# skipperro/selkies-gstreamer

Hardware: AMD Instinct MI355X
Metric: encoded fps + glass-to-glass p50 ms at 1920x1080; concurrent 60fps sessions/node (higher is better)
Workload: dtype uint8 pixels / int32 integer transforms (bit-exact vs CPU reference); 1 GPU; model=H.264 Constrained Baseline CAVLC, striped stripes 64px, CRF 25, global_batch=8, seq_len=1, parallelism=session-parallel dp1 x 8 sessions/GPU, resolution=1920x1080, backend=hip, deblock=auto, me_full=True, upload_overlap=False, frames_in_flight=1, num_refs=1, numa_node_rank0=0

## Files before the change

csrc/kernels/h264_kernels.hip:

```cpp
#include "h264_gpu.h"
#include "../codec/color.h"
#include "../codec/h264_mb.h"
#include "../codec/h264_ep.h"

namespace sk {
namespace h264 {
namespace gpu {

__device__ __forceinline__ int lane_id() { return threadIdx.x & 63; }

__device__ __forceinline__ void wave_sync() {
    __builtin_amdgcn_fence(__ATOMIC_RELEASE, "wavefront");
    __builtin_amdgcn_wave_barrier();
    __builtin_amdgcn_fence(__ATOMIC_ACQUIRE, "wavefront");
}

__device__ __forceinline__ int wave_sum(int v) {
    v += __builtin_amdgcn_mov_dpp(v, 0xB1, 0xF, 0xF, false);
    v += __builtin_amdgcn_mov_dpp(v, 0x4E, 0xF, 0xF, false);
    v += __builtin_amdgcn_mov_dpp(v, 0x124, 0xF, 0xF, false);
    v += __builtin_amdgcn_mov_dpp(v, 0x128, 0xF, 0xF, false);
    return __builtin_amdgcn_readlane(v, 0) + __builtin_amdgcn_readlane(v, 16) +
           __builtin_amdgcn_readlane(v, 32) + __builtin_amdgcn_readlane(v, 48);
}
// ... 822 lines not shown
            const MeResult r = a.me[first + i];
            sad += r.sad;
            dev += r.intra_est;
            ref1 += r.ref == 1;
        }
    }
    if (a.ltr_slots) {
        for (int o = 32; o > 0; o >>= 1) ref1 += __shfl_down(ref1, o);
        if (lane_id() == 0) red1[threadIdx.x >> 6] = ref1;
    }
    for (int o = 32; o > 0; o >>= 1) {
        sad += __shfl_down(sad, o);
        dev += __shfl_down(dev, o);
    }
    if (lane_id() == 0) {
        red[0][threadIdx.x >> 6] = sad;
        red[1][threadIdx.x >> 6] = dev;
    }
    __syncthreads();
    if (threadIdx.x == 0) {
        const long long ts = red[0][0] + red[0][1] + red[0][2] + red[0][3];
        const long long td = red[1][0] + red[1][1] + red[1][2] + red[1][3];
        t.final_action = (p && ts > td) ? ACT_I : t.action;
        if (a.ltr_slots)
            a.ltr_task[s].ref1_mbs = (planned_p && t.final_action == ACT_P) ? red1[0] + red1[1] + red1[2] + red1[3] : 0;
        a.rc_slice[2 * s] = ts;
        a.rc_slice[2 * s + 1] = td;
        a.tasks_host[s] = t;
    }
}

__device__ void rc_qp_serial(const FrameArgs& a, const int* key, RcState& rc, SliceTask* tasks, const long long* sums) {
    const int seq = key[5];
    int plan_qp = a.plan_cfg.qp;
    const int qo = key[1];
    if (qo > 0) plan_qp = qo;
    if (seq != rc.seq) {
        const int mode = key[3];
        const int kbps = key[4];
        const RcState old = rc;
        rc_init(rc, mode, plan_qp, kbps, (float)a.rc_fps, a.W * a.H, old.vbv_ms, old.codec);
        if (old.mode == mode)
            for (int k = 0; k < 2; k++) {
                rc.last_qp[k] = old.last_qp[k];
                rc.last_qpf[k] = old.last_qpf[k];
                rc.last_bits[k] = old.last_bits[k];
                rc.last_cplx[k] = old.last_cplx[k];
            }
        if (old.mode == mode) rc.cplx_ema = old.cplx_ema;
        rc.seq = seq;
    }
    rc.base_qp = plan_qp;
    rc_apply(rc, tasks, sums, sums + 1, a.num_slices, a.mb_w, plan_qp, 2);
}
constexpr int kRcLdsSlices = 128;
__global__ __launch_bounds__(64) void k_rc_qp(FrameArgs a) {
    __shared__ long long sums_l[2 * kRcLdsSlices];
    __shared__ SliceTask tasks_l[kRcLdsSlices];
    __shared__ RcState rc_l;
    __shared__ int key_l[6];
    static_assert(sizeof(RcState) % 4 == 0 && sizeof(SliceTask) % 4 == 0, "dword copies");
    const int ns = a.num_slices, l = threadIdx.x;
    const bool in_lds = ns <= kRcLdsSlices;
    if (in_lds) {
        for (int i = l; i < ns * (int)(sizeof(SliceTask) / 4); i += 64)
            reinterpret_cast<uint32_t*>(tasks_l)[i] = reinterpret_cast<const uint32_t*>(a.tasks)[i];
        for (int i = l; i < 2 * ns; i += 64) sums_l[i] = a.rc_slice[i];
        if (l < (int)(sizeof(RcState) / 4)) reinterpret_cast<uint32_t*>(&rc_l)[l] = reinterpret_cast<const uint32_t*>(a.rc)[l];
        if (l < 6) key_l[l] = a.key_dev[l];
    }
    __syncthreads();
    if (l == 0) {
        if (in_lds) rc_qp_serial(a, key_l, rc_l, tasks_l, sums_l);
        else rc_qp_serial(a, a.key_dev, *a.rc, a.tasks, a.rc_slice);
    }
    __syncthreads();
    if (in_lds) {
        if (l < (int)(sizeof(RcState) / 4)) reinterpret_cast<uint32_t*>(a.rc)[l] = reinterpret_cast<const uint32_t*>(&rc_l)[l];
        for (int s = l; s < ns; s += 64) a.tasks[s].qp = tasks_l[s].qp;
    }
    for (int s = l; s < ns; s += 64) a.tasks_host[s].qp = in_lds ? tasks_l[s].qp : a.tasks[s].qp;
}

__device__ __forceinline__ void rc_account_wave(const FrameArgs& a, const int* sizes, int n, int stride, int per_slice) {
    long long b = 0;
    for (int i = lane_id(); i < n; i += 64)
        if (!per_slice || i % per_slice < slice_nals(a, a.tasks[i / per_slice])) b += sizes[(size_t)i * stride];
    for (int o = 32; o > 0; o >>= 1) b += __shfl_down(b, o);
    if (lane_id() == 0) rc_account(*a.rc, 8 * b);
}

__global__ __launch_bounds__(64) void k_rc_account(FrameArgs a, const int* sizes, int n, int stride, int per_slice) {
    rc_account_wave(a, sizes, n, stride, per_slice);
}

__global__ __launch_bounds__(256) void k_rc_guard(FrameArgs a) {
    __shared__ long long part[4];
    const int tid = threadIdx.x;
    long long b = 0;
    for (int i = tid; i < a.num_slices; i += 256) {
        const int nn = slice_nals(a, a.tasks[i]);
        for (int j = 0; j < nn; j++) b += a.slice_info[4 * (i * a.nal_per_slice + j)];
    }
    for (int o = 32; o > 0; o >>= 1) b += __shfl_down(b, o);
    if ((tid & 63) == 0) part[tid >> 6] = b;
    __syncthreads();
    if (tid != 0) return;
    const long long bits = 8 * (part[0] + part[1] + part[2] + part[3]);
    const int applied = rc_redo_step(*a.rc, bits) ? rc_redo(*a.rc, a.tasks, a.num_slices, bits) : 0;
    *a.rc_redo = applied ? 1 : 0;
    if (applied)
        for (int i = 0; i < a.num_slices; i++) a.tasks_host[i].qp = a.tasks[i].qp;
}

__global__ __launch_bounds__(256) void k_rc_guard_sizes(FrameArgs a, const int* sizes, int n, int* redo, int chained) {
    __shared__ long long part[4];
    if (chained && *redo == 0) return;
    const int tid = threadIdx.x;
    long long b = 0;
    for (int i = tid; i < n; i += 256) b += sizes[i];
    for (int o = 32; o > 0; o >>= 1) b += __shfl_down(b, o);
    if ((tid & 63) == 0) part[tid >> 6] = b;
    __syncthreads();
    if (tid != 0) return;
    const long long bits = 8 * (part[0] + part[1] + part[2] + part[3]);
    const int applied = rc_redo_step(*a.rc, bits) ? rc_redo(*a.rc, a.tasks, a.num_slices, bits) : 0;
    *redo = applied ? 1 : 0;
    if (applied)
        for (int i = 0; i < a.num_slices; i++) a.tasks_host[i].qp = a.tasks[i].qp;
}

struct MbScratch {
    int16_t coef[kCoefPerMb];
    int dcy[16];
    int dcc[8];
    int blk_stat[32];
    int misc[8];
    uint8_t nnz[24];
    uint8_t pad[8];
    int cdcp[8];
    uint8_t nb[64];
    uint8_t nbtr[4];
    uint8_t ref13[32];
    uint8_t ry[256];
};

__device__ __forceinline__ void lds_hadamard4x4(int* x) {
    const int l = lane_id();
    if (l < 4) {
        int a = x[l * 4 + 0], b = x[l * 4 + 1], c = x[l * 4 + 2], d = x[l * 4 + 3];
        int s01 = a + b, d01 = a - b, s23 = c + d, d23 = c - d;
        x[l * 4 + 0] = s01 + s23;
        x[l * 4 + 1] = s01 - s23;
        x[l * 4 + 2] = d01 - d23;
        x[l * 4 + 3] = d01 + d23;
    }
    wave_sync();
    if (l < 4) {
        int a = x[l], b = x[4 + l], c = x[8 + l], d = x[12 + l];
        int s01 = a + b, d01 = a - b, s23 = c + d, d23 = c - d;
        x[l] = s01 + s23;
        x[4 + l] = s01 - s23;
        x[8 + l] = d01 - d23;
        x[12 + l] = d01 + d23;
    }
    wave_sync();
// ... 571 lines not shown
    if (l < 57) {
        const int c = 2 + l % 19, seg = l / 19;
        const int r0 = seg == 0 ? 2 : (seg == 1 ? 9 : 15), n = seg == 0 ? 7 : 6;
        int v[12];
#pragma unroll
        for (int i = 0; i < 12; i++) v[i] = (i < n + 5) ? Q.b1[r0 - 2 + i][c] : 0;
#pragma unroll
        for (int i = 0; i < 7; i++)
            if (i < n)
                Q.jp[r0 + i][c] = (uint8_t)sk_clip255((qtap6(v[i], v[i + 1], v[i + 2], v[i + 3], v[i + 4], v[i + 5]) +
                                                       512) >> 10);
    }
    wave_sync();
}
__device__ __forceinline__ int qpel_lookup(const QpelLds& Q, int x, int y, int dqx, int dqy) {
    const int cx = x + 3 + (dqx >> 2), cy = y + 3 + (dqy >> 2), fx = dqx & 3, fy = dqy & 3;
    const int G = Q.win[cy][cx];
    if (!(fx | fy)) return G;
    if (fy == 0) {
        const int b = Q.bp[cy][cx];
        return fx == 2 ? b : ((fx == 1 ? G : Q.win[cy][cx + 1]) + b + 1) >> 1;
    }
    if (fx == 0) {
        const int h = Q.hp[cy][cx];
        return fy == 2 ? h : ((fy == 1 ? G : Q.win[cy + 1][cx]) + h + 1) >> 1;
    }
    if (fx == 2 && fy == 2) return Q.jp[cy][cx];
    if (fx == 2) return (Q.bp[cy + (fy >> 1)][cx] + Q.jp[cy][cx] + 1) >> 1;
    if (fy == 2) return (Q.hp[cy][cx + (fx >> 1)] + Q.jp[cy][cx] + 1) >> 1;
    return (Q.bp[cy + (fy >> 1)][cx] + Q.hp[cy][cx + (fx >> 1)] + 1) >> 1;
}

__global__ __launch_bounds__(256) void k_subpel(FrameArgs a) {
    __shared__ QpelLds Qw[4];
    QpelLds& Q = Qw[threadIdx.x >> 6];
    const int nmb = a.mb_w * a.mb_h;
    const int idx = xcd_remap(blockIdx.x, gridDim.x) * 4 + (threadIdx.x >> 6);
    if (idx >= nmb) return;
    const int mbx = idx % a.mb_w, mby = idx / a.mb_w;
    const SliceTask t = a.tasks[mby / a.rows_per_slice];
    if (t.final_action != ACT_P) return;
    const MeResult r = a.me[idx];
    const int l = lane_id();
    const int sl = mby / a.rows_per_slice;
    if (r.sad <= kSubpelMinSad || !subpel_gate(t.frame_num, a.plan_state[sl].subpel_prev, t.num_rows * a.mb_w)) {
        if (l == 0) { a.me[idx].fx = 0; a.me[idx].fy = 0; }
        return;
    }
    const int ylo = t.pic_row0 * 16, yhi = (t.pic_row0 + t.pic_rows) * 16 - 1;
    qpel_fill_fast(Q, r.ref ? ref1_planes(a, sl).y : a.ref.y, a.stride_y, a.stride_y, ylo, yhi, mbx * 16 + r.mvx - 3,
              mby * 16 + r.mvy - 3);
    const int yy = l >> 2, xx = 4 * (l & 3);
    const uint32_t sw = *reinterpret_cast<const uint32_t*>(a.src.y + (size_t)(mby * 16 + yy) * a.stride_y +
                                                          mbx * 16 + xx);
    auto sad_q = [&](int dqx, int dqy) __attribute__((always_inline)) {
        int s = 0;
#pragma unroll
        for (int j = 0; j < 4; j++)
            s += sk_abs((int)((sw >> (8 * j)) & 255u) - qpel_lookup(Q, xx + j, yy, dqx, dqy));
        return wave_sum(s);
    };
    int bx = 0, by = 0, best = sad_q(0, 0);
    const int int_sad = best;
    for (int step = 2; step >= 1; step--) {
        const int cx = bx, cy = by;
        for (int k = 0; k < 8; k++) {
            const int kk = k < 4 ? k : k + 1;
            const int qx = cx + step * (kk % 3 - 1), qy = cy + step * (kk / 3 - 1);
            const int c = sad_q(qx, qy);
            if (c < best) {
                best = c;
                bx = qx;
                by = qy;
            }
        }
    }
    if (l == 0) {
        a.me[idx].fx = (int8_t)bx;
        a.me[idx].fy = (int8_t)by;
        if ((bx | by) && subpel_hit(best, int_sad)) atomicAdd(&a.plan_state[mby / a.rows_per_slice].subpel_hits, 1);
    }
}

__global__ __launch_bounds__(256) void k_code_inter(FrameArgs a) {
    if (a.gate && *a.gate == 0) return;
    __shared__ MbScratch Sw[4];
    __shared__ QpelLds Qw[4];
    __shared__ CavlcTables T;
    MbScratch& S = Sw[threadIdx.x >> 6];
    int nmb = a.mb_w * a.mb_h;
    int idx = xcd_remap(blockIdx.x, gridDim.x) * 4 + (threadIdx.x >> 6);
    const bool valid = idx < nmb;
    int mbx = valid ? idx % a.mb_w : 0, mby = valid ? idx / a.mb_w : 0;
    int s = mby / a.rows_per_slice;
    const SliceTask t = a.tasks[s];
    int l = lane_id();
    if (valid && t.final_action == ACT_SKIPALL && l == 0) {
        MbInfo z;
        memset(&z, 0, sizeof(z));
        a.mbs[idx] = z;
        a.me[idx].mvx = 0;
        a.me[idx].mvy = 0;
        a.me[idx].ref = 0;
        a.me[idx].fx = a.me[idx].fy = 0;
    }
    const bool coded = valid && t.final_action == ACT_P;
    if (!__syncthreads_or(coded)) return;
    load_cavlc_tables(T, a.cavlc_tabs);
    __syncthreads();
    if (!coded) return;
    auto nbr = [&](int ox, int oy, bool ok) {
        MvNb n;
        n.avail = ok;
        n.ref = ok ? a.me[oy * a.mb_w + ox].ref : -1;
        n.mvx = ok ? me_qx(a.me[oy * a.mb_w + ox]) : 0;
        n.mvy = ok ? me_qy(a.me[oy * a.mb_w + ox]) : 0;
        return n;
    };
    bool top = mby > t.first_row;
    MvNb A = nbr(mbx - 1, mby, mbx > 0);
    MvNb B = nbr(mbx, mby - 1, top);
    MvNb C = nbr(mbx + 1, mby - 1, top && mbx + 1 < a.mb_w);
    if (!C.avail) C = nbr(mbx - 1, mby - 1, top && mbx > 0);
    const int refi = a.me[idx].ref;
    const Planes rp = refi ? ref1_planes(a, s) : a.ref;
    int pmx, pmy, smx, smy;
    mv_pred16x16(A, B, C, refi, &pmx, &pmy);
    mv_pskip(A, B, C, &smx, &smy);
    int mvx = me_qx(a.me[idx]), mvy = me_qy(a.me[idx]);

    const int b = l >> 2, r = l & 3;
    const int cl = l & 31, comp = cl >> 4, cb = (cl >> 2) & 3;
    int ylo = t.pic_row0 * 16, yhi = (t.pic_row0 + t.pic_rows) * 16 - 1;
    int px = mbx * 16 + blk_x(b) * 4, py = mby * 16 + blk_y(b) * 4 + r;
    uint32_t sw = *reinterpret_cast<const uint32_t*>(a.src.y + (size_t)py * a.stride_y + px);
    int src_l[4], pred_l[4];
    if (!((mvx | mvy) & 3)) {
        int sy = sk_clip(py + (mvy >> 2), ylo, yhi);
        uint32_t pw = load_ref4(rp.y + (size_t)sy * a.stride_y, px + (mvx >> 2), a.stride_y);
#pragma unroll
        for (int j = 0; j < 4; j++) pred_l[j] = (pw >> (8 * j)) & 255;
    } else {
        QpelLds& Q = *reinterpret_cast<QpelLds*>(&Qw[threadIdx.x >> 6]);
        qpel_fill(Q, rp.y, a.stride_y, a.stride_y, ylo, yhi, mbx * 16 + (mvx >> 2) - 3, mby * 16 + (mvy >> 2) - 3);
#pragma unroll
        for (int j = 0; j < 4; j++)
            pred_l[j] = qpel_lookup(Q, px - mbx * 16 + j, py - mby * 16, mvx & 3, mvy & 3);
    }
#pragma unroll
    for (int j = 0; j < 4; j++) src_l[j] = (sw >> (8 * j)) & 255;
    const uint8_t* cs = comp ? a.src.v : a.src.u;
    const uint8_t* crf = comp ? rp.v : rp.u;
    int cx0 = mbx * 8 + (cb & 1) * 4, cy0 = mby * 8 + (cb >> 1) * 4 + r;
    uint32_t csw = *reinterpret_cast<const uint32_t*>(cs + (size_t)cy0 * a.stride_c + cx0);
    int src_c[4], pred_c[4];
    const uint8_t* cbase = crf + (size_t)(t.pic_row0 * 8) * a.stride_c;
#pragma unroll
    for (int j = 0; j < 4; j++) {
        src_c[j] = (csw >> (8 * j)) & 255;
        pred_c[j] = chroma_mc_sample(cbase, a.stride_c, a.stride_c, t.pic_rows * 8, cx0 + j,
                                     cy0 - t.pic_row0 * 8, mvx, mvy);
    }
    MbInfo mb;
    memset(&mb, 0, sizeof(mb));
    mb.type = MB_P_16x16;
    int rec_l[4], rec_c[4];
    code_mb(src_l, pred_l, src_c, pred_c, t.qp, false, S, mb, rec_l, rec_c,
            a.coefs + (size_t)idx * kCoefPerMb, T, nullptr, 0,
            a.aq_strength > 0 ? aq_start_qp(t.qp, a.aq[idx]) : -1);
    uint32_t rw = (uint32_t)rec_l[0] | ((uint32_t)rec_l[1] << 8) | ((uint32_t)rec_l[2] << 16) |
                  ((uint32_t)rec_l[3] << 24);
    *reinterpret_cast<uint32_t*>(a.rec.y + (size_t)py * a.stride_y + px) = rw;
    if (l < 32) {
        uint8_t* cr = comp ? a.rec.v : a.rec.u;
        uint32_t cw = (uint32_t)rec_c[0] | ((uint32_t)rec_c[1] << 8) | ((uint32_t)rec_c[2] << 16) |
                      ((uint32_t)rec_c[3] << 24);
        *reinterpret_cast<uint32_t*>(cr + (size_t)cy0 * a.stride_c + cx0) = cw;
    }
    if (l == 0) {
        mb.mvx = (int16_t)mvx;
        mb.mvy = (int16_t)mvy;
        mb.ref = (uint8_t)refi;
        if (mb.cbp == 0 && refi == 0 && mvx == smx && mvy == smy) {
            mb.type = MB_P_SKIP;
        } else {
            mb.mvdx = (int16_t)(mvx - pmx);
            mb.mvdy = (int16_t)(mvy - pmy);
        }
        for (int i = 0; i < 24; i++) mb.nnz[i] = S.nnz[i];
        a.mbs[idx] = mb;
    }
}

__device__ __forceinline__ void intra_modes_wave(const int* src_l, const int* src_c, const uint8_t* topp, const uint8_t* leftp,
                                 int tl, const uint8_t* const* ctop, const uint8_t* const* cleft, const int* ctl,
                                 bool aT, bool aL, int* cdcp, int* luma_mode, int* chroma_mode,
                                 int* luma_sad = nullptr) {
    const int l = lane_id();
    const int b = l >> 2, r = l & 3;
    const int cl = l & 31, comp = cl >> 4, cb = (cl >> 2) & 3;
    const int lx = blk_x(b) * 4, ly = blk_y(b) * 4 + r;
    int dc = i16_dc(topp, leftp, aT, aL);
    int pa = 0, pb = 0, pc = 0;
    if (aT && aL) i16_plane_params(topp, leftp, tl, &pa, &pb, &pc);
    const int order[4] = {2, 0, 1, 3};
    int best_mode = 2, best_sad = 0x7fffffff;
    for (int oi = 0; oi < 4; oi++) {
        int m = order[oi];
        if ((m == 0 && !aT) || (m == 1 && !aL) || (m == 3 && !(aT && aL))) continue;
        int sad = 0;
#pragma unroll
        for (int j = 0; j < 4; j++)
            sad += sk_abs(src_l[j] - i16_pred_pixel(m, lx + j, ly, topp, leftp, tl, aT, aL, dc, pa, pb, pc));
        sad = wave_sum(sad);
        if (sad < best_sad) { best_sad = sad; best_mode = m; }
    }
    const uint8_t* ct = ctop[comp];
    const uint8_t* cf = cleft[comp];
    const int clx = (cb & 1) * 4, cly = (cb >> 1) * 4 + r;
    int qa = 0, qb = 0, qc = 0;
    if (aT && aL) chroma_plane_params(ct, cf, ctl[comp], &qa, &qb, &qc);
    if (l < 8) cdcp[l] = chroma_dc_block(l & 1, (l >> 1) & 1, ctop[l >> 2], cleft[l >> 2], aT, aL);
    wave_sync();
    const int cdc_mine = cdcp[comp * 4 + cb];
    int best_cm = 0, best_csad = 0x7fffffff;
    for (int m = 0; m < 4; m++) {
        if ((m == 1 && !aL) || (m == 2 && !aT) || (m == 3 && !(aT && aL))) continue;
        int sad = 0;
#pragma unroll
        for (int j = 0; j < 4; j++) {
            int x = clx + j, y = cly, v;
            if (m == 0) v = cdc_mine;
            else if (m == 1) v = cf[y];
            else if (m == 2) v = ct[x];
            else v = sk_clip255((qa + qb * (x - 3) + qc * (y - 3) + 16) >> 5);
            sad += sk_abs(src_c[j] - v);
        }
        sad = wave_sum(l < 32 ? sad : 0);
        if (sad < best_csad) { best_csad = sad; best_cm = m; }
    }
    *luma_mode = best_mode;
    *chroma_mode = best_cm;
    if (luma_sad) *luma_sad = best_sad;
}

__device__ __forceinline__ int wave_sum_masked(int v, bool on) { return wave_sum(on ? v : 0); }

__device__ __forceinline__ void intra_pred_lanes(int mode, int cmode, const uint8_t* nb, int tl, const int* ctl, bool aT, bool aL,
                                 int* pred_l, int* pred_c) {
    const int l = lane_id();
    const int b = l >> 2, r = l & 3;
    const int cl = l & 31, comp = cl >> 4, cb = (cl >> 2) & 3;
    const int lx = blk_x(b) * 4, ly = blk_y(b) * 4 + r;
    const int clx = (cb & 1) * 4, cly = (cb >> 1) * 4 + r;
    const int e = nb[l];
    if (mode == 0) {
#pragma unroll
        for (int j = 0; j < 4; j++) pred_l[j] = nb[lx + j];
    } else if (mode == 1) {
        const int v = nb[16 + ly];
#pragma unroll
        for (int j = 0; j < 4; j++) pred_l[j] = v;
    } else if (mode == 2) {
        const int st = wave_sum_masked(e, l < 16), sl = wave_sum_masked(e, l >= 16 && l < 32);
        const int dc = (aT && aL) ? (st + sl + 16) >> 5 : (aL ? (sl + 8) >> 4 : (aT ? (st + 8) >> 4 : 128));
#pragma unroll
        for (int j = 0; j < 4; j++) pred_l[j] = dc;
    } else {
        const int i = l & 7, base = l < 8 ? 0 : 16;
        const int p1 = nb[base + 8 + i];
        const int p0 = 6 - i >= 0 ? nb[base + sk_max(6 - i, 0)] : tl;
        const int term = (i + 1) * (p1 - p0);
        const int H = wave_sum_masked(term, l < 8), V = wave_sum_masked(term, l >= 8 && l < 16);
        const int pa = 16 * (nb[16 + 15] + nb[15]);
        const int pb = (5 * H + 32) >> 6, pc = (5 * V + 32) >> 6;
#pragma unroll
        for (int j = 0; j < 4; j++) pred_l[j] = sk_clip255((pa + pb * (lx + j - 7) + pc * (ly - 7) + 16) >> 5);
    }
    const int ct = 32 + 8 * comp, cf = 48 + 8 * comp;
    if (cmode == 0) {
        const int q = quad_sum(e);
        const int st = __shfl(q, 32 + 8 * comp + 4 * (cb & 1));
        const int sl = __shfl(q, 48 + 8 * comp + 4 * (cb >> 1));
        const int bx = cb & 1, by = cb >> 1;
        int v;
        if (bx == by) v = (aT && aL) ? (st + sl + 4) >> 3 : (aL ? (sl + 2) >> 2 : (aT ? (st + 2) >> 2 : 128));
        else if (bx == 1) v = aT ? (st + 2) >> 2 : (aL ? (sl + 2) >> 2 : 128);
        else v = aL ? (sl + 2) >> 2 : (aT ? (st + 2) >> 2 : 128);
#pragma unroll
        for (int j = 0; j < 4; j++) pred_c[j] = v;
    } else if (cmode == 1) {
        const int v = nb[cf + cly];
#pragma unroll
        for (int j = 0; j < 4; j++) pred_c[j] = v;
    } else if (cmode == 2) {
#pragma unroll
        for (int j = 0; j < 4; j++) pred_c[j] = nb[ct + clx + j];
    } else {
        const int tc = (l >> 4) & 1, isv = (l >> 3) & 1, i = l & 3;
        const int base = isv ? 48 + 8 * tc : 32 + 8 * tc;
        const int p1 = nb[base + 4 + i];
        const int p0 = 2 - i >= 0 ? nb[base + sk_max(2 - i, 0)] : ctl[tc];
        const int term = (l & 4) ? 0 : (i + 1) * (p1 - p0);
        const int H0 = wave_sum_masked(term, l < 8), V0 = wave_sum_masked(term, l >= 8 && l < 16);
        const int H1 = wave_sum_masked(term, l >= 16 && l < 24), V1 = wave_sum_masked(term, l >= 24 && l < 32);
        const int H = comp ? H1 : H0, V = comp ? V1 : V0;
        const int pa = 16 * (nb[cf + 7] + nb[ct + 7]);
        const int pb = (34 * H + 32) >> 6, pc = (34 * V + 32) >> 6;
#pragma unroll
        for (int j = 0; j < 4; j++) pred_c[j] = sk_clip255((pa + pb * (clx + j - 3) + pc * (cly - 3) + 16) >> 5);
    }
}

__device__ void load_nb_planes(const Planes& P, int sy, int sc, int mbx, int mby, bool aT, bool aL, uint8_t* nb,
                               int* tl, int* ctl) {
    const int l = lane_id();
    int v = 0;
    if (l < 16) v = aT ? P.y[(size_t)(mby * 16 - 1) * sy + mbx * 16 + l] : 0;
    else if (l < 32) v = aL ? P.y[(size_t)(mby * 16 + l - 16) * sy + mbx * 16 - 1] : 0;
    else if (l < 48) {
        const uint8_t* C = (l & 8) ? P.v : P.u;
        v = aT ? C[(size_t)(mby * 8 - 1) * sc + mbx * 8 + (l & 7)] : 0;
    } else {
        const uint8_t* C = (l & 8) ? P.v : P.u;
        v = aL ? C[(size_t)(mby * 8 + (l & 7)) * sc + mbx * 8 - 1] : 0;
    }
    nb[l] = (uint8_t)v;
    *tl = (aT && aL) ? P.y[(size_t)(mby * 16 - 1) * sy + mbx * 16 - 1] : 0;
    ctl[0] = (aT && aL) ? P.u[(size_t)(mby * 8 - 1) * sc + mbx * 8 - 1] : 0;
    ctl[1] = (aT && aL) ? P.v[(size_t)(mby * 8 - 1) * sc + mbx * 8 - 1] : 0;
    wave_sync();
}

__global__ __launch_bounds__(256) void k_intra_prep(FrameArgs a) {
    if (a.gate && *a.gate == 0) return;
    __shared__ MbScratch Sw[4];
    __shared__ CavlcTables T;
    __shared__ uint8_t nb_w[4][64];
    MbScratch& S = Sw[threadIdx.x >> 6];
    uint8_t* nb = nb_w[threadIdx.x >> 6];
    const int nmb = a.mb_w * a.mb_h;
    const int idx = xcd_remap(blockIdx.x, gridDim.x) * 4 + (threadIdx.x >> 6);
    const bool valid = idx < nmb;
    const int mbx = valid ? idx % a.mb_w : 0, mby = valid ? idx / a.mb_w : 0;
    const SliceTask t = a.tasks[mby / a.rows_per_slice];
    const bool coded = valid && t.final_action == ACT_I;
    if (!__syncthreads_or(coded)) return;
    load_cavlc_tables(T, a.cavlc_tabs);
    __syncthreads();
    if (!coded) return;
    const int l = lane_id();
    const int b = l >> 2, r = l & 3;
    const int cl = l & 31, comp = cl >> 4, cb = (cl >> 2) & 3;
    bool aT = mby > t.first_row, aL = mbx > 0;
    if (split_i(a, t)) {
        aT = false;
        aL = aL && (idx - t.first_row * a.mb_w) % kIntraSubMbs != 0;
    }
    int tl, ctl[2];
    load_nb_planes(a.src, a.stride_y, a.stride_c, mbx, mby, aT, aL, nb, &tl, ctl);
    const uint8_t* ctop[2] = {nb + 32, nb + 40};
    const uint8_t* cleft[2] = {nb + 48, nb + 56};
    int px = mbx * 16 + blk_x(b) * 4, py = mby * 16 + blk_y(b) * 4 + r;
    uint32_t sw = *reinterpret_cast<const uint32_t*>(a.src.y + (size_t)py * a.stride_y + px);
    const uint8_t* cs = comp ? a.src.v : a.src.u;
    int cx0 = mbx * 8 + (cb & 1) * 4, cy0 = mby * 8 + (cb >> 1) * 4 + r;
    uint32_t csw = *reinterpret_cast<const uint32_t*>(cs + (size_t)cy0 * a.stride_c + cx0);
    int src_l[4], src_c[4];
#pragma unroll
    for (int j = 0; j < 4; j++) {
        src_l[j] = (sw >> (8 * j)) & 255;
        src_c[j] = (csw >> (8 * j)) & 255;
    }
    int mode, cmode, sad16;
    intra_modes_wave(src_l, src_c, nb, nb + 16, tl, ctop, cleft, ctl, aT, aL, S.cdcp, &mode, &cmode, &sad16);
    int pred_l[4], pred_c[4];
    intra_pred_lanes(mode, cmode, nb, tl, ctl, aT, aL, pred_l, pred_c);
    const int start = a.aq_strength > 0 ? aq_start_qp(t.qp, a.aq[idx]) : -1;
    MbInfo cand;
    memset(&cand, 0, sizeof(cand));
    bool i4 = false;
    const bool aTR = aT && mbx + 1 < a.mb_w;
    auto src_smp = [&](int x, int y) __attribute__((always_inline)) -> int {
        return a.src.y[(size_t)(mby * 16 + y) * a.stride_y + mbx * 16 + x];
    };
    if (a.intra4x4) {
        const int q = l >> 2;
        int* sads = reinterpret_cast<int*>(S.coef);
        uint8_t* refs = S.ry;
        for (int k = r; k < 13; k += 4) refs[q * 13 + k] = (uint8_t)i4_ref_sample(src_smp, q, aT, aL, aTR, k);
        wave_sync();
        const I4RefView ref{refs + q * 13, i4_has_top(q, aT), i4_has_left(q, aL)};
        for (int m = 0; m < 9; m++) {
            int sad = 0;
#pragma unroll
            for (int j = 0; j < 4; j++) sad += sk_abs(src_l[j] - i4_pred_px(m, ref, j, r));
            sad = quad_sum(sad);
            if (r == 0) sads[q * 9 + m] = i4_mode_ok(m, ref.hasT, ref.hasL) ? sad : -1;
        }
        wave_sync();
        const int lam = i4_lambda(t.qp);
        int total = 0;
        for (int b = 0; b < 16; b++) {
            const int bx = blk_x(b), by = blk_y(b);
            const int ma = bx > 0 ? i4_mode(cand, blk_from_xy(bx - 1, by)) : (aL ? 2 : -1);
            const int mt = by > 0 ? i4_mode(cand, blk_from_xy(bx, by - 1)) : (aT ? 2 : -1);
            const int pm = i4_predicted(ma, mt);
            int best = 0x7fffffff, bm = I4_DC;
            for (int m = 0; m < 9; m++) {
                const int sd = sads[b * 9 + m];
                if (sd < 0) continue;
                const int cost = sd + lam * (m == pm ? 1 : 4);
                if (cost < best) { best = cost; bm = m; }
            }
            set_i4_mode(cand, b, bm);
            total += best;
        }
        i4 = i4_wins(total, sad16, t.qp);
        wave_sync();
    }
    MbInfo mb;
    memset(&mb, 0, sizeof(mb));
    int qp;
    if (i4) {
        mb.type = MB_I4x4;
        mb.chroma_mode = (uint8_t)cmode;
        mb.i4lo = cand.i4lo;
        mb.i4hi = cand.i4hi;
        int rec_l[4], rec_c[4];
        qp = code_mb_i4(src_smp, src_l, src_c, pred_c, start >= 0 ? start : t.qp, t.qp, aT, aL, aTR, S, mb, rec_l,
                        rec_c, nullptr, T);
    } else {
        int rec_l[4], rec_c[4];
        qp = code_mb(src_l, pred_l, src_c, pred_c, t.qp, true, S, mb, rec_l, rec_c, nullptr, T, nullptr, 0, start,
                     true);
    }
    if (l == 0) {
        MbInfo o;
        memset(&o, 0, sizeof(o));
        o.type = i4 ? MB_I4x4 : MB_I16x16;
        o.i16_mode = (uint8_t)mode;
        o.chroma_mode = (uint8_t)cmode;
        o.qp = (uint8_t)qp;
        o.i4lo = cand.i4lo;
        o.i4hi = cand.i4hi;
        a.mbs[idx] = o;
    }
}

constexpr int kMaxRows = 16;
struct IntraEdges {
    uint8_t bot_y[kMaxRows][4][16];
    uint8_t bot_c[kMaxRows][4][2][8];
    uint8_t right_y[kMaxRows][16];
    uint8_t right_c[kMaxRows][2][8];
};

struct IntraSrc {
    uint32_t y[64];
    uint32_t c[32];
    int mode, cmode, qp, i4;
    uint32_t i4m[2];
};
constexpr int kIntraRing = 4;

template <int MAXROWS>
__global__ __launch_bounds__(64 * (MAXROWS + 1)) void k_code_intra(FrameArgs a) {
    if (a.gate && *a.gate == 0) return;
    __shared__ MbScratch Sw[MAXROWS];
    __shared__ IntraEdges E;
    __shared__ IntraSrc R[MAXROWS][kIntraRing];
    __shared__ uint8_t zero16[16];
    __shared__ CavlcTables T;
    int s = blockIdx.x;
    const SliceTask t = a.tasks[s];
    if (t.final_action != ACT_I || split_i(a, t)) return;
#ifdef SK_STAMPS
    const unsigned long long t_start = __builtin_amdgcn_s_memrealtime();
    const unsigned long long c_start = __builtin_amdgcn_s_memtime();
    if (a.dbg && blockIdx.x == 0 && (threadIdx.x & 63) == 0)
        a.dbg[1024 + 128 + (threadIdx.x >> 6)] = (unsigned)__builtin_amdgcn_s_getreg((31 << 11) | 4);
#endif
    if (threadIdx.x < 16) zero16[threadIdx.x] = 0;
    load_cavlc_tables(T, a.cavlc_tabs);
    int w = threadIdx.x >> 6;
    int l = lane_id();
    const int rows = t.num_rows;
    const int steps = a.mb_w + 2 * (rows - 1);
    const bool producer = w == MAXROWS;
    auto produce = [&](int st) {
        for (int row = 0; row < rows; row++) {
            const int x = st - 2 * row;
            if (x < 0 || x >= a.mb_w) continue;
            const int my = t.first_row + row;
            IntraSrc& d = R[row][x & (kIntraRing - 1)];
            d.y[l] = *reinterpret_cast<const uint32_t*>(a.src.y + (size_t)(my * 16 + (l >> 2)) * a.stride_y + x * 16 +
                                                        4 * (l & 3));
            if (l < 32) {
                const uint8_t* P = (l >> 4) ? a.src.v : a.src.u;
                d.c[l] = *reinterpret_cast<const uint32_t*>(P + (size_t)(my * 8 + ((l >> 1) & 7)) * a.stride_c +
                                                            x * 8 + 4 * (l & 1));
            }
            if (l == 0) {
                const MbInfo pre = a.mbs[my * a.mb_w + x];
                d.mode = pre.i16_mode;
                d.cmode = pre.chroma_mode;
                d.qp = pre.qp;
                d.i4 = pre.type == MB_I4x4;
                d.i4m[0] = pre.i4lo;
                d.i4m[1] = pre.i4hi;
            }
        }
    };
    if (producer) {
        __builtin_amdgcn_s_setprio(2);
        produce(0);
        produce(1);
    }
    __syncthreads();
#ifdef SK_STAMPS
    const unsigned long long c_loop = __builtin_amdgcn_s_memtime();
#endif
    if (!producer) __builtin_amdgcn_s_setprio(3);
    MbScratch& S = Sw[producer ? 0 : w];
    const int b = l >> 2, r = l & 3;
    const int cl = l & 31, comp = cl >> 4, cb = (cl >> 2) & 3;
    const int lx = blk_x(b) * 4, ly = blk_y(b) * 4 + r;
    const int clx = (cb & 1) * 4, cly = (cb >> 1) * 4 + r;
    const int mby = t.first_row + w;
    for (int step = 0; step < steps; step++) {
// ... 884 lines not shown
                    }
                    return __builtin_amdgcn_ubfe(e < 2 ? w01 : w23, 16 * (e & 1) + bsh, 4);
                };
                const uint32_t p_left = chroma ? e1.w : e1.x, p_top = chroma ? e2.x : e1.y;
                const uint32_t p_in = chroma ? e2.y : e1.z;
                uint32_t* own = ring[r][sl][0];
                if (emask & 15u) {
                    uint32_t* lp = ring[r][(x - 1) & (kSlots - 1)][act ? l : 0];
                    uint32_t* op = own + 4 * (act ? l : 0);
                    int v[20];
                    unpack4((emask & 1u) ? lp[ldw] : 0u, v);
#pragma unroll
                    for (int q = 0; q < 4; q++) unpack4(op[q], v + 4 + 4 * q);
#pragma unroll
                    for (int e = 0; e < 4; e++)
                        if (emask & (1u << e)) {
                            const int bs = act ? bs_of(e0.x, e0.y, e) : 0;
                            if (e == 0) db_filter_line<true>(v, bs, p_left, chroma);
                            else db_filter_line<false>(v + 4 * e, bs, p_in, chroma);
                        }
                    if (act) {
                        if (emask & 1u) lp[ldw] = pack4(v);
#pragma unroll
                        for (int q = 0; q < 4; q++) op[q] = pack4(v + 4 + 4 * q);
                    }
                    wave_sync();
                }
                if (emask & 0xF0u) {
                    uint8_t* ob = reinterpret_cast<uint8_t*>(own) + lbase * 16 + li;
                    uint8_t* tb = reinterpret_cast<uint8_t*>(ring[sk_max(r - 1, 0)][sl][0]) +
                                  (lbase + nrows - 4) * 16 + li;
                    const bool top_on = (emask & 16u) && act;
                    int v[20];
#pragma unroll
                    for (int q = 0; q < 4; q++) v[q] = top_on ? tb[q * 16] : 0;
#pragma unroll
                    for (int q = 0; q < 16; q++) v[4 + q] = act ? ob[sk_min(q, nrows - 1) * 16] : 0;
#pragma unroll
                    for (int e = 0; e < 4; e++)
                        if (emask & (16u << e)) {
                            const int bs = act ? bs_of(e0.z, e0.w, e) : 0;
                            if (e == 0) db_filter_line<true>(v, bs, p_top, chroma);
                            else db_filter_line<false>(v + 4 * e, bs, p_in, chroma);
                        }
                    if (act) {
                        if (top_on) {
#pragma unroll
                            for (int q = 1; q < 4; q++) tb[q * 16] = (uint8_t)v[q];
                        }
#pragma unroll
                        for (int q = 0; q < 16; q++)
                            if (q < nrows) ob[q * 16] = (uint8_t)v[4 + q];
                    }
                    wave_sync();
                }
            }
            const int xb = x - 3;
            if (act && xb >= 0 && xb < W) {
                const uint4 q = *reinterpret_cast<const uint4*>(ring[r][xb & (kSlots - 1)][l]);
                uint8_t* p0 = dst + rowoff + xb * mbbytes;
                *reinterpret_cast<uint2*>(p0) = make_uint2(q.x, q.y);
                *reinterpret_cast<uint2*>(p0 + half2) = chroma ? make_uint2(q.x, q.y) : make_uint2(q.z, q.w);
            }
        }
        lds_barrier();
    }
}

void launch_convert_damage(const FrameArgs& a, hipStream_t s) {
    dim3 grid((a.mb_w + 15) / 16, a.mb_h);
    if (a.yuv_fmt) hipLaunchKernelGGL(k_yuv_damage, grid, dim3(256), 0, s, a);
    else hipLaunchKernelGGL(k_convert_damage, grid, dim3(256), 0, s, a);
}

void launch_frontend(const FrameArgs& a, hipStream_t s) {
    int nmb = a.mb_w * a.mb_h;
    hipLaunchKernelGGL(k_plan, dim3(1), dim3(256), 0, s, a);
    if (a.ltr_slots) {
        hipLaunchKernelGGL(k_ltr_match, dim3(a.rows_per_slice, 1 + a.ltr_slots, a.num_slices), dim3(256), 0, s, a);
        hipLaunchKernelGGL(k_ltr_decide, dim3(1), dim3(256), 0, s, a);
    }
    if (a.me_full) hipLaunchKernelGGL(k_me, dim3((nmb + 3) / 4), dim3(256), 0, s, a);
    else hipLaunchKernelGGL(k_motion_search, dim3(nmb), dim3(64), 0, s, a);
    hipLaunchKernelGGL(k_decide, dim3(a.num_slices), dim3(256), 0, s, a);
    hipLaunchKernelGGL(k_rc_qp, dim3(1), dim3(64), 0, s, a);
    if (a.subpel) hipLaunchKernelGGL(k_subpel, dim3((nmb + 3) / 4), dim3(256), 0, s, a);
}

void launch_rc_guard_sizes(const FrameArgs& a, const int* sizes, int n, int* redo, bool chained, hipStream_t s) {
    hipLaunchKernelGGL(k_rc_guard_sizes, dim3(1), dim3(256), 0, s, a, sizes, n, redo, chained ? 1 : 0);
}

void launch_rc_account(const FrameArgs& a, const int* sizes, int n, int stride, int per_slice, hipStream_t s) {
    hipLaunchKernelGGL(k_rc_account, dim3(1), dim3(64), 0, s, a, sizes, n, stride, per_slice);
}

static void launch_code(const FrameArgs& a, hipStream_t s) {
    int nmb = a.mb_w * a.mb_h;
    hipLaunchKernelGGL(k_code_inter, dim3((nmb + 3) / 4), dim3(256), 0, s, a);
    hipLaunchKernelGGL(k_intra_prep, dim3((nmb + 3) / 4), dim3(256), 0, s, a);
    if (a.nal_per_slice > 1)
        hipLaunchKernelGGL(k_code_intra_sub, dim3((a.num_slices * a.nal_per_slice + 3) / 4), dim3(256), 0, s, a);
    else if (a.rows_per_slice <= 4)
        hipLaunchKernelGGL(k_code_intra<4>, dim3(a.num_slices), dim3(64 * 5), 0, s, a);
    else
        hipLaunchKernelGGL(k_code_intra<kMaxRows - 1>, dim3(a.num_slices), dim3(64 * kMaxRows), 0, s, a);
    hipLaunchKernelGGL(k_cavlc, dim3((nmb + 3) / 4), dim3(256), 0, s, a);
}

void launch_encode(const FrameArgs& a, hipStream_t s, bool guard) {
    int nmb = a.mb_w * a.mb_h;
    launch_frontend(a, s);
    if (a.aq_strength > 0) hipLaunchKernelGGL(k_aq, dim3((nmb + 3) / 4), dim3(256), 0, s, a);
    launch_code(a, s);
    if (guard && a.rc_redo) {
        hipLaunchKernelGGL(k_slice_pack<true>, dim3(a.num_slices), dim3(kPackThreads), 0, s, a);
        hipLaunchKernelGGL(k_rc_guard, dim3(1), dim3(256), 0, s, a);
        FrameArgs b = a;
        b.gate = a.rc_redo;
        launch_code(b, s);
    }
    hipLaunchKernelGGL(k_slice_pack<false>, dim3(a.num_slices), dim3(kPackThreads), 0, s, a);
}

void launch_commit(const FrameArgs& a, hipStream_t s, bool filter, bool account) {
    hipLaunchKernelGGL(k_commit, dim3((a.mb_w + 15) / 16, a.mb_h), dim3(256), 0, s, a, account ? 1 : 0);
    if (a.deblock && filter) {
        const int nmb = a.mb_w * a.mb_h;
        hipLaunchKernelGGL(k_deblock_prep, dim3((nmb + 3) / 4), dim3(256), 0, s, a);
        hipLaunchKernelGGL(k_deblock_edges, dim3((nmb + 255) / 256), dim3(256), 0, s, a);
        if (a.rows_per_slice <= 4)
            hipLaunchKernelGGL(k_deblock<4>, dim3(a.num_slices), dim3(64 * a.rows_per_slice), 0, s, a);
        else
            hipLaunchKernelGGL(k_deblock<kMaxRows>, dim3(a.num_slices), dim3(64 * a.rows_per_slice), 0, s, a);
    }
}

}
}
}
```

Before: 5933 frames/s (1920x1080 H.264, all sessions, all GPUs).

## Fuse slice decide with rate-control QP and merge intra prep into inter kernel

Adds a single-block k_decide_qp kernel that loads all motion results and slice tasks into registers and LDS, reduces per-slice SAD, intra estimate and ref1 counts with wave-level accumulation, and then runs the serial rate-control QP pass. It replaces the separate k_decide and k_rc_qp launches when the frame fits in 8192 MBs. It also folds k_intra_prep into k_code_inter, so one launch handles both P and I macroblocks, with the intra neighbour buffer reusing the QpelLds space. The aim is fewer kernel launches and less global traffic per frame. The cost is a single-block reduction over the whole frame, and higher LDS and register pressure in the merged coding kernel, which may reduce occupancy.

New measurement: 5974 frames/s (1920x1080 H.264, all sessions, all GPUs), median of 6. About the same (+0.7%).

```diff
diff --git a/csrc/kernels/h264_kernels.hip b/csrc/kernels/h264_kernels.hip
--- a/csrc/kernels/h264_kernels.hip
+++ b/csrc/kernels/h264_kernels.hip
@@ -928,6 +928,141 @@
     for (int s = l; s < ns; s += 64) a.tasks_host[s].qp = in_lds ? tasks_l[s].qp : a.tasks[s].qp;
 }
 
+constexpr int kDecideQpThreads = 512;
+constexpr int kDecideQpLoads = 16;
+constexpr int kDecideQpMaxMbs = kDecideQpThreads * kDecideQpLoads;
+__global__ __launch_bounds__(kDecideQpThreads) void k_decide_qp(FrameArgs a) {
+    __shared__ long long sums_l[2 * kRcLdsSlices];
+    __shared__ int ref1_l[kRcLdsSlices];
+    __shared__ SliceTask tasks_l[kRcLdsSlices];
+    __shared__ RcState rc_l;
+    __shared__ int key_l[6];
+    static_assert(sizeof(MeResult) == 16 && sizeof(RcState) % 4 == 0 && sizeof(SliceTask) % 4 == 0, "dword / uint4 copies");
+    const int ns = a.num_slices, tid = threadIdx.x, l = lane_id(), nmb = a.mb_w * a.mb_h;
+    const int task_words = ns * (int)(sizeof(SliceTask) / 4), rc_words = (int)(sizeof(RcState) / 4);
+    if (ns > kRcLdsSlices) {
+        for (int s = tid >> 6; s < ns; s += kDecideQpThreads / 64) {
+            SliceTask& t = a.tasks[s];
+            const bool planned_p = t.action == ACT_P;
+            long long sad = 0, dev = 0;
+            int ref1 = 0;
+            if (planned_p || t.action == ACT_I) {
+                const int first = t.first_row * a.mb_w, n = t.num_rows * a.mb_w;
+                for (int i = l; i < n; i += 64) {
+                    const MeResult r = a.me[first + i];
+                    sad += r.sad;
+                    dev += r.intra_est;
+                    ref1 += r.ref == 1;
+                }
+            }
+            for (int o = 32; o > 0; o >>= 1) {
+                sad += __shfl_down(sad, o);
+                dev += __shfl_down(dev, o);
+                ref1 += __shfl_down(ref1, o);
+            }
+            if (l == 0) {
+                t.final_action = (planned_p && t.allow_scenecut && sad > dev) ? ACT_I : t.action;
+                if (a.ltr_slots) a.ltr_task[s].ref1_mbs = (planned_p && t.final_action == ACT_P) ? ref1 : 0;
+                a.rc_slice[2 * s] = sad;
+                a.rc_slice[2 * s + 1] = dev;
+            }
+        }
+        __syncthreads();
+        if (tid == 0) rc_qp_serial(a, a.key_dev, *a.rc, a.tasks, a.rc_slice);
+        __syncthreads();
+        for (int i = tid; i < task_words; i += kDecideQpThreads)
+            reinterpret_cast<uint32_t*>(a.tasks_host)[i] = reinterpret_cast<const uint32_t*>(a.tasks)[i];
+        return;
+    }
+    constexpr int kTaskLoads = kRcLdsSlices * (int)(sizeof(SliceTask) / 4) / kDecideQpThreads;
+    static_assert(kTaskLoads * kDecideQpThreads == kRcLdsSlices * (int)(sizeof(SliceTask) / 4), "task dwords per thread");
+    uint32_t tv[kTaskLoads];
+#pragma unroll
+    for (int k = 0; k < kTaskLoads; k++)
+        tv[k] = reinterpret_cast<const uint32_t*>(a.tasks)[sk_min(k * kDecideQpThreads + tid, task_words - 1)];
+    const uint32_t rcv = reinterpret_cast<const uint32_t*>(a.rc)[sk_min(tid, rc_words - 1)];
+    const int keyv = a.key_dev[sk_min(tid, 5)];
+    const int mb0 = (tid >> 6) * (64 * kDecideQpLoads) + l;
+    uint4 m[kDecideQpLoads];
+#pragma unroll
+    for (int k = 0; k < kDecideQpLoads; k++)
+        m[k] = reinterpret_cast<const uint4*>(a.me)[sk_min(mb0 + 64 * k, nmb - 1)];
+#pragma unroll
+    for (int k = 0; k < kTaskLoads; k++)
+        if (k * kDecideQpThreads + tid < task_words) reinterpret_cast<uint32_t*>(tasks_l)[k * kDecideQpThreads + tid] = tv[k];
+    if (tid < rc_words) reinterpret_cast<uint32_t*>(&rc_l)[tid] = rcv;
+    if (tid < 6) key_l[tid] = keyv;
+    for (int i = tid; i < ns; i += kDecideQpThreads) {
+        sums_l[2 * i] = sums_l[2 * i + 1] = 0;
+        ref1_l[i] = 0;
+    }
+    __syncthreads();
+    const int smb = a.mb_w * a.rows_per_slice;
+    const float rsmb = 1.0f / (float)smb;
+    int cur = -1, acc_s = 0, acc_d = 0, acc_r = 0;
+    auto flush = [&]() __attribute__((always_inline)) {
+        if (cur >= 0) {
+            const int ws = wave_sum(acc_s), wd = wave_sum(acc_d), wr = wave_sum(acc_r);
+            if (l == 0) {
+                atomicAdd(reinterpret_cast<unsigned long long*>(&sums_l[2 * cur]), (unsigned long long)ws);
+                atomicAdd(reinterpret_cast<unsigned long long*>(&sums_l[2 * cur + 1]), (unsigned long long)wd);
+                atomicAdd(&ref1_l[cur], wr);
+            }
+        }
+        cur = -1;
+        acc_s = acc_d = acc_r = 0;
+    };
+#pragma unroll
+    for (int k = 0; k < kDecideQpLoads; k++) {
+        const int i = mb0 + 64 * k;
+        if (i - l >= nmb) break;
+        const bool valid = i < nmb;
+        int s = (int)((float)i * rsmb);
+        const int rem = i - s * smb;
+        s += (rem >= smb) - (rem < 0);
+        if (!valid) s = -1;
+        const int act = valid ? tasks_l[s].action : ACT_NONE;
+        const bool on = act == ACT_P || act == ACT_I;
+        const int sad = on ? (int)m[k].y : 0, dev = on ? (int)m[k].z : 0;
+        const int ref1 = on && (int16_t)(m[k].w & 0xffffu) == 1;
+        const int s0 = __builtin_amdgcn_readfirstlane(s);
+        if (__all(!valid || s == s0)) {
+            if (s0 != cur) {
+                flush();
+                cur = s0;
+            }
+            acc_s += sad;
+            acc_d += dev;
+            acc_r += ref1;
+        } else {
+            flush();
+            if (on) {
+                atomicAdd(reinterpret_cast<unsigned long long*>(&sums_l[2 * s]), (unsigned long long)sad);
+                atomicAdd(reinterpret_cast<unsigned long long*>(&sums_l[2 * s + 1]), (unsigned long long)dev);
+                atomicAdd(&ref1_l[s], ref1);
+            }
+        }
+    }
+    flush();
+    __syncthreads();
+    for (int s = tid; s < ns; s += kDecideQpThreads) {
+        SliceTask& t = tasks_l[s];
+        const bool planned_p = t.action == ACT_P;
+        t.final_action = (planned_p && t.allow_scenecut && sums_l[2 * s] > sums_l[2 * s + 1]) ? ACT_I : t.action;
+        if (a.ltr_slots) a.ltr_task[s].ref1_mbs = (planned_p && t.final_action == ACT_P) ? ref1_l[s] : 0;
+    }
+    __syncthreads();
+    if (tid == 0) rc_qp_serial(a, key_l, rc_l, tasks_l, sums_l);
+    __syncthreads();
+    for (int i = tid; i < task_words; i += kDecideQpThreads) {
+        const uint32_t v = reinterpret_cast<const uint32_t*>(tasks_l)[i];
+        reinterpret_cast<uint32_t*>(a.tasks)[i] = v;
+        reinterpret_cast<uint32_t*>(a.tasks_host)[i] = v;
+    }
+    if (tid < rc_words) reinterpret_cast<uint32_t*>(a.rc)[tid] = reinterpret_cast<const uint32_t*>(&rc_l)[tid];
+    for (int i = tid; i < 2 * ns; i += kDecideQpThreads) a.rc_slice[i] = sums_l[i];
+}
+
 __device__ __forceinline__ void rc_account_wave(const FrameArgs& a, const int* sizes, int n, int stride, int per_slice) {
     long long b = 0;
     for (int i = lane_id(); i < n; i += 64)
@@ -1665,33 +1800,9 @@
     }
 }
 
-__global__ __launch_bounds__(256) void k_code_inter(FrameArgs a) {
-    if (a.gate && *a.gate == 0) return;
-    __shared__ MbScratch Sw[4];
-    __shared__ QpelLds Qw[4];
-    __shared__ CavlcTables T;
-    MbScratch& S = Sw[threadIdx.x >> 6];
-    int nmb = a.mb_w * a.mb_h;
-    int idx = xcd_remap(blockIdx.x, gridDim.x) * 4 + (threadIdx.x >> 6);
-    const bool valid = idx < nmb;
-    int mbx = valid ? idx % a.mb_w : 0, mby = valid ? idx / a.mb_w : 0;
-    int s = mby / a.rows_per_slice;
-    const SliceTask t = a.tasks[s];
-    int l = lane_id();
-    if (valid && t.final_action == ACT_SKIPALL && l == 0) {
-        MbInfo z;
-        memset(&z, 0, sizeof(z));
-        a.mbs[idx] = z;
-        a.me[idx].mvx = 0;
-        a.me[idx].mvy = 0;
-        a.me[idx].ref = 0;
-        a.me[idx].fx = a.me[idx].fy = 0;
-    }
-    const bool coded = valid && t.final_action == ACT_P;
-    if (!__syncthreads_or(coded)) return;
-    load_cavlc_tables(T, a.cavlc_tabs);
-    __syncthreads();
-    if (!coded) return;
+__device__ __forceinline__ void code_inter_mb(const FrameArgs& a, const SliceTask& t, int s, int idx, int mbx, int mby,
+                                              MbScratch& S, QpelLds& Q, const CavlcTables& T) {
+    const int l = lane_id();
     auto nbr = [&](int ox, int oy, bool ok) {
         MvNb n;
         n.avail = ok;
@@ -1724,7 +1835,6 @@
 #pragma unroll
         for (int j = 0; j < 4; j++) pred_l[j] = (pw >> (8 * j)) & 255;
     } else {
-        QpelLds& Q = *reinterpret_cast<QpelLds*>(&Qw[threadIdx.x >> 6]);
         qpel_fill(Q, rp.y, a.stride_y, a.stride_y, ylo, yhi, mbx * 16 + (mvx >> 2) - 3, mby * 16 + (mvy >> 2) - 3);
 #pragma unroll
         for (int j = 0; j < 4; j++)
@@ -1798,12 +1908,12 @@
         sad = wave_sum(sad);
         if (sad < best_sad) { best_sad = sad; best_mode = m; }
     }
-    const uint8_t* ct = ctop[comp];
-    const uint8_t* cf = cleft[comp];
+    const uint8_t* ct = comp ? ctop[1] : ctop[0];
+    const uint8_t* cf = comp ? cleft[1] : cleft[0];
     const int clx = (cb & 1) * 4, cly = (cb >> 1) * 4 + r;
     int qa = 0, qb = 0, qc = 0;
-    if (aT && aL) chroma_plane_params(ct, cf, ctl[comp], &qa, &qb, &qc);
-    if (l < 8) cdcp[l] = chroma_dc_block(l & 1, (l >> 1) & 1, ctop[l >> 2], cleft[l >> 2], aT, aL);
+    if (aT && aL) chroma_plane_params(ct, cf, comp ? ctl[1] : ctl[0], &qa, &qb, &qc);
+    if (l < 8) cdcp[l] = chroma_dc_block(l & 1, (l >> 1) & 1, (l >> 2) ? ctop[1] : ctop[0], (l >> 2) ? cleft[1] : cleft[0], aT, aL);
     wave_sync();
     const int cdc_mine = cdcp[comp * 4 + cb];
     int best_cm = 0, best_csad = 0x7fffffff;
@@ -1883,7 +1993,7 @@
         const int tc = (l >> 4) & 1, isv = (l >> 3) & 1, i = l & 3;
         const int base = isv ? 48 + 8 * tc : 32 + 8 * tc;
         const int p1 = nb[base + 4 + i];
-        const int p0 = 2 - i >= 0 ? nb[base + sk_max(2 - i, 0)] : ctl[tc];
+        const int p0 = 2 - i >= 0 ? nb[base + sk_max(2 - i, 0)] : (tc ? ctl[1] : ctl[0]);
         const int term = (l & 4) ? 0 : (i + 1) * (p1 - p0);
         const int H0 = wave_sum_masked(term, l < 8), V0 = wave_sum_masked(term, l >= 8 && l < 16);
         const int H1 = wave_sum_masked(term, l >= 16 && l < 24), V1 = wave_sum_masked(term, l >= 24 && l < 32);
@@ -1895,7 +2005,7 @@
     }
 }
 
-__device__ void load_nb_planes(const Planes& P, int sy, int sc, int mbx, int mby, bool aT, bool aL, uint8_t* nb,
+__device__ __forceinline__ void load_nb_planes(const Planes& P, int sy, int sc, int mbx, int mby, bool aT, bool aL, uint8_t* nb,
                                int* tl, int* ctl) {
     const int l = lane_id();
     int v = 0;
@@ -1915,23 +2025,8 @@
     wave_sync();
 }
 
-__global__ __launch_bounds__(256) void k_intra_prep(FrameArgs a) {
-    if (a.gate && *a.gate == 0) return;
-    __shared__ MbScratch Sw[4];
-    __shared__ CavlcTables T;
-    __shared__ uint8_t nb_w[4][64];
-    MbScratch& S = Sw[threadIdx.x >> 6];
-    uint8_t* nb = nb_w[threadIdx.x >> 6];
-    const int nmb = a.mb_w * a.mb_h;
-    const int idx = xcd_remap(blockIdx.x, gridDim.x) * 4 + (threadIdx.x >> 6);
-    const bool valid = idx < nmb;
-    const int mbx = valid ? idx % a.mb_w : 0, mby = valid ? idx / a.mb_w : 0;
-    const SliceTask t = a.tasks[mby / a.rows_per_slice];
-    const bool coded = valid && t.final_action == ACT_I;
-    if (!__syncthreads_or(coded)) return;
-    load_cavlc_tables(T, a.cavlc_tabs);
-    __syncthreads();
-    if (!coded) return;
+__device__ __forceinline__ void intra_prep_mb(const FrameArgs& a, const SliceTask& t, int idx, int mbx, int mby,
+                                              MbScratch& S, uint8_t* nb, const CavlcTables& T) {
     const int l = lane_id();
     const int b = l >> 2, r = l & 3;
     const int cl = l & 31, comp = cl >> 4, cb = (cl >> 2) & 3;
@@ -1984,10 +2079,12 @@
         wave_sync();
         const int lam = i4_lambda(t.qp);
         int total = 0;
+        uint64_t m16 = 0;
+        auto mode_of = [&](int blk) { return (int)((m16 >> (4 * blk)) & 15u); };
         for (int b = 0; b < 16; b++) {
             const int bx = blk_x(b), by = blk_y(b);
-            const int ma = bx > 0 ? i4_mode(cand, blk_from_xy(bx - 1, by)) : (aL ? 2 : -1);
-            const int mt = by > 0 ? i4_mode(cand, blk_from_xy(bx, by - 1)) : (aT ? 2 : -1);
+            const int ma = bx > 0 ? mode_of(blk_from_xy(bx - 1, by)) : (aL ? 2 : -1);
+            const int mt = by > 0 ? mode_of(blk_from_xy(bx, by - 1)) : (aT ? 2 : -1);
             const int pm = i4_predicted(ma, mt);
             int best = 0x7fffffff, bm = I4_DC;
             for (int m = 0; m < 9; m++) {
@@ -1996,9 +2093,11 @@
                 const int cost = sd + lam * (m == pm ? 1 : 4);
                 if (cost < best) { best = cost; bm = m; }
             }
-            set_i4_mode(cand, b, bm);
+            m16 |= (uint64_t)bm << (4 * b);
             total += best;
         }
+        cand.i4lo = (uint32_t)m16;
+        cand.i4hi = (uint32_t)(m16 >> 32);
         i4 = i4_wins(total, sad16, t.qp);
         wave_sync();
     }
@@ -2029,6 +2128,37 @@
         o.i4hi = cand.i4hi;
         a.mbs[idx] = o;
     }
+}
+
+__global__ __launch_bounds__(256) void k_code_inter(FrameArgs a) {
+    if (a.gate && *a.gate == 0) return;
+    __shared__ MbScratch Sw[4];
+    __shared__ QpelLds Qw[4];
+    __shared__ CavlcTables T;
+    static_assert(sizeof(QpelLds) >= 64, "intra_prep_mb's neighbour samples live in the wave's QpelLds");
+    MbScratch& S = Sw[threadIdx.x >> 6];
+    int nmb = a.mb_w * a.mb_h;
+    int idx = xcd_remap(blockIdx.x, gridDim.x) * 4 + (threadIdx.x >> 6);
+    const bool valid = idx < nmb;
+    int mbx = valid ? idx % a.mb_w : 0, mby = valid ? idx / a.mb_w : 0;
+    int s = mby / a.rows_per_slice;
+    const SliceTask t = a.tasks[s];
+    int l = lane_id();
+    if (valid && t.final_action == ACT_SKIPALL && l == 0) {
+        MbInfo z;
+        memset(&z, 0, sizeof(z));
+        a.mbs[idx] = z;
+        a.me[idx].mvx = 0;
+        a.me[idx].mvy = 0;
+        a.me[idx].ref = 0;
+        a.me[idx].fx = a.me[idx].fy = 0;
+    }
+    const bool inter = valid && t.final_action == ACT_P, prep = valid && t.final_action == ACT_I;
+    if (!__syncthreads_or(inter || prep)) return;
+    load_cavlc_tables(T, a.cavlc_tabs);
+    __syncthreads();
+    if (inter) code_inter_mb(a, t, s, idx, mbx, mby, S, Qw[threadIdx.x >> 6], T);
+    else if (prep) intra_prep_mb(a, t, idx, mbx, mby, S, reinterpret_cast<uint8_t*>(&Qw[threadIdx.x >> 6]), T);
 }
 
 constexpr int kMaxRows = 16;
@@ -3079,8 +3209,12 @@
     }
     if (a.me_full) hipLaunchKernelGGL(k_me, dim3((nmb + 3) / 4), dim3(256), 0, s, a);
     else hipLaunchKernelGGL(k_motion_search, dim3(nmb), dim3(64), 0, s, a);
-    hipLaunchKernelGGL(k_decide, dim3(a.num_slices), dim3(256), 0, s, a);
-    hipLaunchKernelGGL(k_rc_qp, dim3(1), dim3(64), 0, s, a);
+    if (nmb <= kDecideQpMaxMbs) {
+        hipLaunchKernelGGL(k_decide_qp, dim3(1), dim3(kDecideQpThreads), 0, s, a);
+    } else {
+        hipLaunchKernelGGL(k_decide, dim3(a.num_slices), dim3(256), 0, s, a);
+        hipLaunchKernelGGL(k_rc_qp, dim3(1), dim3(64), 0, s, a);
+    }
     if (a.subpel) hipLaunchKernelGGL(k_subpel, dim3((nmb + 3) / 4), dim3(256), 0, s, a);
 }
 
@@ -3095,7 +3229,6 @@
 static void launch_code(const FrameArgs& a, hipStream_t s) {
     int nmb = a.mb_w * a.mb_h;
     hipLaunchKernelGGL(k_code_inter, dim3((nmb + 3) / 4), dim3(256), 0, s, a);
-    hipLaunchKernelGGL(k_intra_prep, dim3((nmb + 3) / 4), dim3(256), 0, s, a);
     if (a.nal_per_slice > 1)
         hipLaunchKernelGGL(k_code_intra_sub, dim3((a.num_slices * a.nal_per_slice + 3) / 4), dim3(256), 0, s, a);
     else if (a.rows_per_slice <= 4)
```
